# maltezfaria/LevelSetMethods.jl

Measured on AMD Instinct MI355X. Metric: Mcells/s per RK3 step (WENO5 advect+reinit), 512^3 fp64; HBM GB/s vs peak, higher is better.
Workload: dtype f64; 1 GPU; 3D 512^3 vortex-deformation WENO5 advection + EikonalReinitializationTerm, RK3, NeumannBC, fp64; cells=134217728, integrator=RK3, arithmetic_mode=fast, parallelism=single, halo_overlap=n/a, prewarm_steps=10, exchange=n/a

## Files before the change

levelsetmethods.jl_amd/csrc/lsm_api.hip:

```cpp
#include <cmath>
#include <cstdio>
#include <cstdlib>
#include <algorithm>
#include <array>
#include <atomic>
#include <chrono>
#include <cstring>
#include <string>
#include <vector>

#include "lsm_internal.h"

namespace lsm {
int launch_stage_fast_1d(const Combo&, const StageArgs&, hipStream_t);
int launch_stage_fast_2d(const Combo&, const StageArgs&, hipStream_t);
int launch_stage_fast_3d(const Combo&, const StageArgs&, hipStream_t);
int launch_stage_strict_1d(const Combo&, const StageArgs&, hipStream_t);
int launch_stage_strict_2d(const Combo&, const StageArgs&, hipStream_t);
int launch_stage_strict_3d(const Combo&, const StageArgs&, hipStream_t);

bool combo_available(const Combo& c) {
    static const int tab[][4] = {{1, 0, 0, 0}, {2, 0, 0, 0}, {0, 1, 0, 0}, {0, 0, 1, 0}, {0, 0, 0, 1}, {0, 0, 0, 2},
                                 {2, 0, 0, 2}, {2, 0, 0, 1}, {0, 1, 1, 0}, {2, 0, 1, 0}, {2, 1, 0, 0}};
    for (auto& t : tab)
// ... 458 lines not shown
            case LSM_TERM_CURVATURE: if (c.curv) goto flush; trial.curv = 1; slot = SLOT_CURV; break;
            case LSM_TERM_EIKONAL: if (c.eik) goto flush; trial.eik = tm.s0 ? 1 : 2; slot = SLOT_EIK; break;
            default: return fail(h, LSM_ERR_INVALID, "lsm_stage: bad term kind");
            }
            if (!combo_available(trial)) break;
            c = trial;
            a.order[cnt++] = slot;
            if (slot == SLOT_ADV) { int r = check_coeff(h, tm.coeff, N); if (r) return r; fill_coeff(tm.coeff, t_stage, a.adv); a.adv_scheme = tm.scheme; }
            if (slot == SLOT_NM) { int r = check_coeff(h, tm.coeff, 1); if (r) return r; fill_coeff(tm.coeff, t_stage, a.nm); }
            if (slot == SLOT_CURV) { int r = check_coeff(h, tm.coeff, 1); if (r) return r; fill_coeff(tm.coeff, t_stage, a.curv); }
            if (slot == SLOT_EIK) a.s0 = (const double*)tm.s0;
            ++i;
        }
    flush:
        if (cnt == 0) return fail(h, LSM_ERR_INVALID, "lsm_stage: internal planner error");
        a.nterms = cnt;
        a.natural = 1;
        for (int k = 1; k < cnt; ++k)
            if (a.order[k] <= a.order[k - 1]) a.natural = 0;
        a.psi = (const double*)psi;
        a.out = (double*)out;
        a.out2 = (double*)out2;
        a.cdt = cdt; a.cdt2 = cdt2;
        a.mb = mb; a.me = me;
        if (first) { a.base_mode = base_mode; a.phin = (const double*)(base_mode == LSM_BASE_PSI ? psi : phin); a.out2_accum = 0; }
        else       { a.base_mode = LSM_BASE_OTHER; a.phin = (const double*)out; a.out2_accum = 1; }
        switch (a.base_mode) {
        case LSM_BASE_PSI: a.base_a = 0.0; a.base_b = 1.0; break;
        case LSM_BASE_RK3_S2: a.base_a = 0.75; a.base_b = 0.25; break;
        case LSM_BASE_RK3_S3: a.base_a = 1.0 / 3; a.base_b = 2.0 / 3; break;
        default: a.base_a = 1.0; a.base_b = 0.0; break;
        }
        hipEvent_t e0 = nullptr, e1 = nullptr;
        const bool timed = h->prof && (h->prof_seen++ % (unsigned long long)h->prof_every) == 0;
        if (timed) { int r = profile_pair(h, &e0, &e1); if (r) return r; LSM_HIP(h, hipEventRecord(e0, s)); }
        int r;
        if (h->mode == LSM_MODE_STRICT)
            r = N == 1 ? launch_stage_strict_1d(c, a, s) : (N == 2 ? launch_stage_strict_2d(c, a, s) : launch_stage_strict_3d(c, a, s));
        else
            r = N == 1 ? launch_stage_fast_1d(c, a, s) : (N == 2 ? launch_stage_fast_2d(c, a, s) : launch_stage_fast_3d(c, a, s));
        if (r) return fail(h, LSM_ERR_INVALID, "lsm_stage: kernel combination not instantiated");
        if (timed) LSM_HIP(h, hipEventRecord(e1, s));
        first = false;
    }
    LSM_HIP(h, hipGetLastError());
    return LSM_OK;
// ... 1342 lines not shown
```

levelsetmethods.jl_amd/csrc/lsm_internal.h:

```cpp
#pragma once
#include <hip/hip_runtime.h>
#include <stdint.h>
#include "../../include/lsm.h"

namespace lsm {

__device__ __forceinline__ double ld_val(const void* p, long long i, int f32) {
    return f32 ? (double)static_cast<const float*>(p)[i] : static_cast<const double*>(p)[i];
}
__device__ __forceinline__ void st_val(void* p, long long i, int f32, double v) {
    if (f32) static_cast<float*>(p)[i] = (float)v;
    else static_cast<double*>(p)[i] = v;
}

struct LsmTuning {
    int stage_tail;
    int stage_tail_dyn;
    int stage_mc;
    int stage_mc2;
    int pairs;
    int stage_generic;
    int xredirect;
    int mredirect;
    int ghost_full_depth;
// ... 23 lines not shown
};

struct StageArgs {
    int n[3];
    int goff[3];
    int gn[3];
    long long s1, s2;
    long long origin;
    double lc[3];
    double h[3];
    double h2[3];
    double inv_h[3];
    double inv_h2[3];
    double dxmin;
    int uniform_h;
    const double* psi;
    const double* phin;
    double* out;
    double* out2;
    int base_mode;
    double base_a, base_b;
    int out2_accum;
    double cdt, cdt2;
    int nterms;
    int order[NSLOTS];
    int natural;
    int adv_scheme;
    CoeffArgs adv, nm, curv;
    const double* s0;
    unsigned nb[3];
    int mb, me;
    int mc;
    unsigned nbig;
    int mc_tail;
    unsigned* tail_ctr;
    unsigned tail_wgs;
    unsigned* tail_ring;
    unsigned* tail_slot_host;
    int xredirect;
    int xkind[2];
    int yredirect;
    int ykind[2];
    int mredirect[2];
    const unsigned char* mask;
    const unsigned char* tile_active;
    const int* tile_list;
// ... 168 lines not shown
```

levelsetmethods.jl_amd/csrc/stage_brick.h:

```cpp
#pragma once
#include "stage_kernel.h"

namespace lsm {
namespace LSM_NS {

template <class LT>
struct LdsElems {
    const LT* p;
    LSM_DEV double operator[](int i) const { return (double)p[i]; }
};
template <int W, int HW, class LT>
struct BrickView {
    LdsElems<LT> T0;
    double c;
    LSM_DEV double z(int k) const { return T0[k * HW]; }
    template <int D>
    LSM_DEV double at(int k) const { return T0[k * (D == 0 ? 1 : (D == 1 ? W : HW))]; }
    template <int A, int B>
    LSM_DEV double corner(int sa, int sb) const { return T0[sa * (A == 0 ? 1 : W) + sb * (B == 1 ? W : HW)]; }
};

#ifndef LSM_BRICK_PITCH
#define LSM_BRICK_PITCH 44
#endif
// ... 90 lines not shown
            const int j = __builtin_ctz(bits);
            bits &= bits - 1;
            nodes[pos++] = (unsigned short)(code0 + j);
        }
    }
#pragma unroll
    for (int k = 0; k < NIT; ++k)
        if (crow < RPI && crow + k * RPI < NROW) vbrick[(crow + k * RPI) * PSEG + cseg] = v[k];
    __syncthreads();
    const long long po = a.origin + (long long)zb * sm + (long long)by0 * sy + bx0;
    PlaneTab pt;
#pragma unroll
    for (int k = 0; k < 3; ++k) pt.adv[k] = pt.nm[k] = pt.curv[k] = 1.0;
    for (int b0 = wv * 64; b0 < N; b0 += NT) {
        const int i = b0 + lane;
        const bool on = i < N;
        const unsigned code = nodes[on ? i : N - 1];
        const int x = code & 31, y = (code >> 5) & 7, z = code >> 8;
        const int l = ((z + G) * H + (y + G)) * WP + x + XL;
        const unsigned eo = (unsigned)z * (unsigned)sm + (unsigned)y * (unsigned)sy + (unsigned)x;
        const NodeIO io{po, (unsigned)sizeof(ST) * eo, 8u * eo, zb + z + a.goff[2]};
        double pre_adv[3] = {0, 0, 0}, pre_nm[3] = {0, 0, 0}, pre_curv[3] = {0, 0, 0};
        const int gi0 = bx0 + x + a.goff[0], gi1 = by0 + y + a.goff[1];
        if constexpr (ADV != 0) coeff_prep<NDIM, NDIM, ADV_SCALED, AK>(a.adv, a, gi0, gi1, pre_adv);
        if constexpr (NM != 0) coeff_prep<NDIM, 1, false, LSM_COEFF_CONST>(a.nm, a, gi0, gi1, pre_nm);
        if constexpr (CURV != 0) coeff_prep<NDIM, 1, false, LSM_COEFF_CONST>(a.curv, a, gi0, gi1, pre_curv);
        NodeOps op;
        node_operands<NDIM, ADV, NM, CURV, EIK, ST, AK>(a, io, pre_adv, pre_nm, pre_curv, pt, op);
        const BrickView<WP, HW, ST> nv{{brick + l}, (double)brick[l]};
        double r1 = 0.0, r2 = 0.0;
        node_update<NDIM, ADV, NM, CURV, EIK, G, WP, ST, true>(a, nv, op, r1, r2);
        node_store<ST, true>(a, io, on, r1, r2);
    }
}

inline bool bricks_applicable(int ADV, int NM, int CURV, const StageArgs& a) {
    if (!a.tune->band_bricks) return false;
    if (!a.mask || !a.brick_list || a.mc <= 0 || a.nbrick_list == 0 || a.out2 || !a.natural || a.xredirect || a.yredirect) return false;
    if ((NM && a.nm.kind != LSM_COEFF_CONST) || (CURV && a.curv.kind != LSM_COEFF_CONST)) return false;
    const int ak = ADV ? a.adv.kind : (int)LSM_COEFF_CONST;
    if (ak != LSM_COEFF_CONST && ak != LSM_COEFF_ROTATION) return false;
    if (a.me <= a.mb || a.tune->stage_generic) return false;
    const long long seg = a.f32 ? 4 : 2, lead = a.origin - LSM_GHOST * a.s2 - LSM_GHOST * a.s1;
    if (lead < BrickCfg::XL || lead % seg || a.s1 % 8 || a.s2 % 8 || a.origin % 8) return false;
    if (((unsigned long long)a.psi | (unsigned long long)a.mask) % 16ull) return false;
    if ((long long)(16 + 2 * LSM_GHOST + 1) * a.s2 * 8 >= (1ll << 31)) return false;
    return true;
}

template <int ADV, int NM, int CURV, int EIK>
int launch_bricks(const StageArgs& a, hipStream_t s) {
    if (!bricks_applicable(ADV, NM, CURV, a)) return -1;
    const int ak = ADV ? a.adv.kind : (int)LSM_COEFF_CONST;
    StageArgs b = a;
    b.nb[0] = (a.n[0] + BrickCfg::TX - 1) / BrickCfg::TX;
    b.nb[1] = (a.n[1] + BrickCfg::TY - 1) / BrickCfg::TY;
    b.nb[2] = (a.me - a.mb + a.mc - 1) / a.mc;
    b.nbig = 0; b.mc_tail = 0; b.tail_wgs = 0;
    constexpr int bz = 8;
    const unsigned sub_per = (unsigned)((a.mc + bz - 1) / bz);
    const unsigned nwg = a.nbrick_list * sub_per;
    const dim3 grid(((nwg + 7u) / 8u) * 8u);
#define LSM_BRICK(STT, AKK, NTT, BZZ) hipLaunchKernelGGL((brick_kernel<ADV, NM, CURV, EIK, STT, AKK, NTT, BZZ>), grid, dim3(NTT), 0, s, b, sub_per)
#define LSM_BRICK_ST(AKK) do { if (!b.f32) LSM_BRICK(double, AKK, 512, 8); else LSM_BRICK(float, AKK, 256, 8); } while (0)
    if constexpr (ADV != 0) {
// ... 11 lines not shown
```

levelsetmethods.jl_amd/csrc/stage_kernel.h:

```cpp
#pragma once
#include <cstdlib>
#include <type_traits>
#include "lsm_internal.h"
#include "stage_math.h"

namespace lsm {
namespace LSM_NS {

#if LSM_STRICT
constexpr bool ADV_SCALED = false;
#else
constexpr bool ADV_SCALED = true;
#endif

constexpr int halo_of(int ADV, int NM, int CURV, int EIK) {
    int g = 0;
    if (ADV == 2) g = 3;
    if (ADV == 1 && g < 1) g = 1;
    if ((NM || EIK) && g < 2) g = 2;
    if (CURV && g < 1) g = 1;
    return g;
}

template <class T>
LSM_DEV T* uniform_ptr(T* p) {
    const unsigned long long v = reinterpret_cast<unsigned long long>(p);
    const unsigned lo = __builtin_amdgcn_readfirstlane((unsigned)v), hi = __builtin_amdgcn_readfirstlane((unsigned)(v >> 32));
    return reinterpret_cast<T*>(((unsigned long long)hi << 32) | lo);
}
LSM_DEV double ld_uniform(const double* t, int i) {
    typedef const __attribute__((address_space(4))) double* cptr;
    return *((cptr)(unsigned long long)t + i);
}
typedef unsigned lsm_v2u __attribute__((ext_vector_type(2)));
LSM_DEV __amdgpu_buffer_rsrc_t plane_rsrc(const void* base, int range = (int)0x80000000u) {
    return __builtin_amdgcn_make_buffer_rsrc(const_cast<void*>(base), 0, range, 0x00020000);
// ... 17 lines not shown
        x = __builtin_bit_cast(double, lsm_v2u{v.x, v.y});
        y = __builtin_bit_cast(double, lsm_v2u{v.z, v.w});
    } else {
        const unsigned long long u = __builtin_bit_cast(unsigned long long, __builtin_amdgcn_raw_buffer_load_b64(plane_rsrc(base, range), boff, 0, AUX));
        x = (double)__builtin_bit_cast(float, (unsigned)u);
        y = (double)__builtin_bit_cast(float, (unsigned)(u >> 32));
    }
}
template <class ST, int AUX = 0>
LSM_DEV void stg2(ST* base, unsigned boff, double x, double y) {
    if constexpr (sizeof(ST) == 8) {
        const lsm_v2u a = __builtin_bit_cast(lsm_v2u, x), b = __builtin_bit_cast(lsm_v2u, y);
        __builtin_amdgcn_raw_buffer_store_b128(lsm_v4u{a.x, a.y, b.x, b.y}, plane_rsrc(base), boff, 0, AUX);
    } else {
        const unsigned long long u = (unsigned long long)__builtin_bit_cast(unsigned, (float)x) | ((unsigned long long)__builtin_bit_cast(unsigned, (float)y) << 32);
        __builtin_amdgcn_raw_buffer_store_b64(__builtin_bit_cast(lsm_v2u, u), plane_rsrc(base), boff, 0, AUX);
    }
}
LSM_DEV unsigned ldg_u8(const unsigned char* base, unsigned boff, int range) {
    return __builtin_amdgcn_raw_buffer_load_b8(
        __builtin_amdgcn_make_buffer_rsrc(const_cast<unsigned char*>(base), 0, __builtin_amdgcn_readfirstlane(range), 0x00020000), boff, 0, 0);
}

template <int NDIM, int NCOMP, bool SCALED = false, int KIND = -1>
LSM_DEV void coeff_prep(const CoeffArgs& c, const StageArgs& a, int gi0, int gi1, double pre[3]) {
    pre[0] = pre[1] = pre[2] = 0.0;
    const int kind = KIND >= 0 ? KIND : c.kind;
    if (kind == LSM_COEFF_CONST) {
#pragma unroll
        for (int k = 0; k < NCOMP; ++k) pre[k] = SCALED ? c.v[k] * a.inv_h[k] : c.v[k];
    } else if (kind == LSM_COEFF_ROTATION) {
        const double x1 = a.lc[0] + (double)gi0 * a.h[0];
        pre[1] = c.v[0] * (x1 - c.v[1]);
        if (SCALED) pre[1] = pre[1] * a.inv_h[1];
        if (NDIM == 3) {
            const double x2 = a.lc[1] + (double)gi1 * a.h[1];
            pre[0] = -(c.v[0] * (x2 - c.v[2]));
            if (SCALED) pre[0] = pre[0] * a.inv_h[0];
        }
    } else if (kind == LSM_COEFF_SEPARABLE) {
#pragma unroll
        for (int k = 0; k < NCOMP; ++k) {
            const double* T = c.sep[k];
            double p = T[gi0];
            if (NDIM == 3) p = p * T[a.gn[0] + gi1];
            pre[k] = SCALED ? p * (c.tfac * a.inv_h[k]) : p;
        }
    }
}
template <int NDIM, int NCOMP, bool SCALED = false, int KIND = -1>
LSM_DEV void coeff_eval(const CoeffArgs& c, const StageArgs& a, const double pre[3], const double tz[3], int gim, long long plane_off,
                        unsigned ocol, double out[3]) {
    const int kind = KIND >= 0 ? KIND : c.kind;
    if (kind == LSM_COEFF_CONST) {
#pragma unroll
        for (int k = 0; k < NCOMP; ++k) out[k] = pre[k];
    } else if (kind == LSM_COEFF_ROTATION) {
        if (NDIM == 2) {
            const double x2 = a.lc[1] + (double)gim * a.h[1];
            out[0] = -(c.v[0] * (x2 - c.v[2]));
            if (SCALED) out[0] = out[0] * a.inv_h[0];
        } else {
            out[0] = pre[0];
        }
        if (NCOMP > 1) out[1] = pre[1];
        if (NCOMP > 2) out[2] = 0.0;
    } else if (kind == LSM_COEFF_SEPARABLE) {
#pragma unroll
        for (int k = 0; k < NCOMP; ++k) {
            double p = pre[k];
            if (NDIM > 1) p = p * tz[k];
            out[k] = SCALED ? p : p * c.tfac;
        }
    } else {
#pragma unroll
        for (int k = 0; k < NCOMP; ++k) {
            out[k] = ldg(uniform_ptr(c.f[k] + plane_off), ocol);
            if (SCALED) out[k] = out[k] * a.inv_h[k];
        }
    }
}

struct PlaneTab {
    double adv[3], nm[3], curv[3];
};
template <int NDIM, int NCOMP, int KIND>
LSM_DEV void plane_tab_one(const CoeffArgs& c, const StageArgs& a, int gim, double tz[3]) {
    tz[0] = tz[1] = tz[2] = 1.0;
    if (NDIM > 1 && (KIND >= 0 ? KIND : c.kind) == LSM_COEFF_SEPARABLE) {
#pragma unroll
        for (int k = 0; k < NCOMP; ++k) tz[k] = ld_uniform(c.sep[k], (NDIM == 3 ? a.gn[0] + a.gn[1] : a.gn[0]) + gim);
    }
}
template <int NDIM, int ADV, int NM, int CURV, int AK>
LSM_DEV void plane_tab(const StageArgs& a, int gim, PlaneTab& t) {
    if constexpr (ADV != 0) plane_tab_one<NDIM, NDIM, AK>(a.adv, a, gim, t.adv);
    if constexpr (NM != 0) plane_tab_one<NDIM, 1, (AK >= 0 ? (int)LSM_COEFF_CONST : -1)>(a.nm, a, gim, t.nm);
    if constexpr (CURV != 0) plane_tab_one<NDIM, 1, (AK >= 0 ? (int)LSM_COEFF_CONST : -1)>(a.curv, a, gim, t.curv);
}

struct NodeIO {
    long long plane_off;
    unsigned ocol;
    unsigned ocold;
    int gim;
};

struct NodeOps {
    double u[3];
    double vnm;
    double bcurv;
    double s0;
    double phin;
    double out2;
    bool have_negs;
    unsigned long long negs[3];
};
template <int NDIM, int ADV, int NM, int CURV, int EIK, class ST, int AK>
LSM_DEV void node_operands(const StageArgs& a, const NodeIO& io, const double pre_adv[3], const double pre_nm[3],
                           const double pre_curv[3], const PlaneTab& pt, NodeOps& op) {
    op.u[0] = op.u[1] = op.u[2] = 0.0;
    op.vnm = op.bcurv = op.s0 = op.phin = op.out2 = 0.0;
    op.have_negs = false;
    if constexpr (ADV != 0) coeff_eval<NDIM, NDIM, ADV_SCALED, AK>(a.adv, a, pre_adv, pt.adv, io.gim, io.plane_off, io.ocold, op.u);
    if constexpr (NM != 0) {
        double vv[3];
        coeff_eval<NDIM, 1, false, (AK >= 0 ? (int)LSM_COEFF_CONST : -1)>(a.nm, a, pre_nm, pt.nm, io.gim, io.plane_off, io.ocold, vv);
        op.vnm = vv[0];
    }
    if constexpr (CURV != 0) {
        double bb[3];
        coeff_eval<NDIM, 1, false, (AK >= 0 ? (int)LSM_COEFF_CONST : -1)>(a.curv, a, pre_curv, pt.curv, io.gim, io.plane_off, io.ocold, bb);
        op.bcurv = bb[0];
    }
    if constexpr (EIK == 1) op.s0 = ldg(uniform_ptr(a.s0 + io.plane_off), io.ocold);
    op.phin = ldg<ST, 0>(uniform_ptr(reinterpret_cast<const ST*>(a.phin) + io.plane_off), io.ocol,
                  __builtin_amdgcn_readfirstlane(a.base_mode == LSM_BASE_PSI ? 0 : (int)0x80000000u));
    if (AK < 0 && a.out2 && a.out2_accum) op.out2 = ldg(uniform_ptr(reinterpret_cast<const ST*>(a.out2) + io.plane_off), io.ocol);
}

template <int NDIM, int G, int W, int R = 0, int RN = 0>
struct NodeView {
    const double* T0;
    const double* Tm;
    const double* Tp;
    const double* zl;
    double c;
// ... 10 lines not shown
        else {
            const double* P = sb > 0 ? Tp : Tm;
            if constexpr (A == 0) return P[sa];
            else return P[sa * W];
        }
    }
};

#if !LSM_STRICT
LSM_DEV double sel64(int m, double x, double y) {
    return __hiloint2double((__double2hiint(x) & m) | (__double2hiint(y) & ~m), (__double2loint(x) & m) | (__double2loint(y) & ~m));
}
#ifndef LSM_NO_UNIFORM_PATHS
#define LSM_UNIFORM_PATHS 1
#else
#define LSM_UNIFORM_PATHS 0
#endif
template <int NDIM, int D, int G, int W, bool PQ, class NV>
LSM_DEV double weno_term(const NV& nv, const StageArgs& a, double v, bool have_negs, unsigned long long negs_known, double& P, double& Q) {
    const double epsf = 1.0e-99 * a.h2[D];
    auto lds = [&](auto Sc) {
        constexpr int ss = (D == 0 ? 1 : W) * decltype(Sc)::value;
        const double q0 = nv.T0[-3 * ss], q1 = nv.T0[-2 * ss], q2 = nv.T0[-ss], q4 = nv.T0[ss], q5 = nv.T0[2 * ss];
        return weno5_undivided_pq<PQ>(q1 - q0, q2 - q1, nv.c - q2, q4 - nv.c, q5 - q4, epsf, P, Q);
    };
    auto reg = [&](auto Sc) {
        constexpr int ss = decltype(Sc)::value;
        return weno5_undivided_pq<PQ>(nv.z(-2 * ss) - nv.z(-3 * ss), nv.z(-ss) - nv.z(-2 * ss), nv.c - nv.z(-ss),
                                      nv.z(ss) - nv.c, nv.z(2 * ss) - nv.z(ss), epsf, P, Q);
    };
    constexpr bool IN_LDS = D == 0 || (D == 1 && NDIM == 3);
    double w;
    const unsigned long long negs = have_negs ? negs_known : __builtin_amdgcn_ballot_w64(__double2hiint(v) < 0);
    if (LSM_UNIFORM_PATHS && negs == 0) {
        if constexpr (IN_LDS) w = lds(std::integral_constant<int, 1>{});
        else w = reg(std::integral_constant<int, 1>{});
    } else if (LSM_UNIFORM_PATHS && negs == __builtin_amdgcn_ballot_w64(true)) {
        if constexpr (IN_LDS) w = lds(std::integral_constant<int, -1>{});
        else w = reg(std::integral_constant<int, -1>{});
    } else {
        const int m = ~(__double2hiint(v) >> 31);
        double q[6];
        if constexpr (IN_LDS) {
            constexpr int st = D == 0 ? 1 : W;
            const int ss = (st & m) | (-st & ~m);
            q[0] = nv.T0[-3 * ss]; q[1] = nv.T0[-2 * ss]; q[2] = nv.T0[-ss];
            q[3] = nv.c;
            q[4] = nv.T0[ss]; q[5] = nv.T0[2 * ss];
        } else {
            q[0] = sel64(m, nv.z(-3), nv.z(3));
            q[1] = sel64(m, nv.z(-2), nv.z(2));
            q[2] = sel64(m, nv.z(-1), nv.z(1));
            q[3] = nv.c;
            q[4] = sel64(m, nv.z(1), nv.z(-1));
            q[5] = sel64(m, nv.z(2), nv.z(-2));
        }
        w = weno5_undivided_pq<PQ>(q[1] - q[0], q[2] - q[1], q[3] - q[2], q[4] - q[3], q[5] - q[4], epsf, P, Q);
    }
    return __builtin_fabs(v) * w;
}
#endif

template <int NDIM, int D, int G, int W, class NV>
LSM_DEV double weno_dim(const NV& nv, const StageArgs& a, double v) {
    const bool up = v > 0;
    double q[6];
    if constexpr (D == 0 || (D == 1 && NDIM == 3)) {
        constexpr int st = D == 0 ? 1 : W;
        const int ss = up ? st : -st;
        q[0] = nv.T0[-3 * ss]; q[1] = nv.T0[-2 * ss]; q[2] = nv.T0[-ss];
        q[3] = nv.c;
        q[4] = nv.T0[ss]; q[5] = nv.T0[2 * ss];
    } else {
        q[0] = up ? nv.z(-3) : nv.z(3);
        q[1] = up ? nv.z(-2) : nv.z(2);
        q[2] = up ? nv.z(-1) : nv.z(1);
        q[3] = nv.c;
        q[4] = up ? nv.z(1) : nv.z(-1);
        q[5] = up ? nv.z(2) : nv.z(-2);
    }
    const double hs = up ? a.h[D] : -a.h[D];
    const double ihs = up ? a.inv_h[D] : -a.inv_h[D];
    return weno5_upwind(q, hs, ihs, 1.0e-99 * a.h2[D]);
}

template <int NDIM, int ADV, int NM, int CURV, int EIK, int G, int W, class ST, bool PLAIN, class NV>
LSM_DEV void node_update(const StageArgs& a, const NV& nv, const NodeOps& op, double& r_out, double& r_out2) {
    const double c = nv.c;
    double Ladv = 0.0, Lnm = 0.0, Lcurv = 0.0, Leik = 0.0;
    double A[3] = {0, 0, 0}, B[3] = {0, 0, 0};
#if LSM_STRICT
    constexpr bool ENO_FROM_WENO = false;
#else
    constexpr bool ENO_FROM_WENO = ADV == 2 && (NM || EIK);
#endif

    if constexpr (ADV != 0) {
        const double* u = op.u;
        auto one = [&](auto Dc) {
            constexpr int D = decltype(Dc)::value;
            const double v = u[D];
            double der;
            if constexpr (ADV == 2) {
#if LSM_STRICT
                der = weno_dim<NDIM, D, G, W>(nv, a, v);
#else
                return weno_term<NDIM, D, G, W, ENO_FROM_WENO>(nv, a, v, op.have_negs, op.negs[D], A[D], B[D]);
#endif
            } else {
#if LSM_STRICT
                der = v > 0 ? (c - nv.template at<D>(-1)) / a.h[D] : (nv.template at<D>(1) - c) / a.h[D];
#else
                der = v > 0 ? (c - nv.template at<D>(-1)) : (nv.template at<D>(1) - c);
#endif
            }
            return v * der;
        };
        Ladv = one(std::integral_constant<int, 0>{});
        if constexpr (NDIM > 1) Ladv = Ladv + one(std::integral_constant<int, 1>{});
        if constexpr (NDIM > 2) Ladv = Ladv + one(std::integral_constant<int, 2>{});
    }

    if constexpr ((NM || EIK) && !ENO_FROM_WENO) {
        auto pr = [&](auto Dc) {
            constexpr int D = decltype(Dc)::value;
            eno2_pair(nv.template at<D>(-2), nv.template at<D>(-1), c, nv.template at<D>(1), nv.template at<D>(2), a.h[D],
                      a.h2[D], a.inv_h[D], A[D], B[D]);
        };
        pr(std::integral_constant<int, 0>{});
        if constexpr (NDIM > 1) pr(std::integral_constant<int, 1>{});
// ... 108 lines not shown
        if constexpr (NDIM > 1) { q4 = q4 + g1; lap = lap + Sd[1]; diag = __builtin_fma(g1, Sd[1], diag); cross = (Gd[0] * Gd[1]) * M01; }
        if constexpr (NDIM > 2) {
            q4 = q4 + g2; lap = lap + Sd[2]; diag = __builtin_fma(g2, Sd[2], diag);
            cross = __builtin_fma(Gd[0] * Gd[2], M02, cross);
            cross = __builtin_fma(Gd[1] * Gd[2], M12, cross);
        }
        const double num = __builtin_fma(lap, q4, -__builtin_fma(0.5, cross, diag));
        Lcurv = q4 < thr ? 0.0 : (bb[0] * scale) * (num * fast_rcp(q4));
#endif
    }

    if constexpr (EIK != 0) {
        const double s = EIK == 1 ? op.s0 : c;
#if LSM_STRICT
        const bool vpos = s > 0;
        double mA = 0.0, mB = 0.0;
#pragma unroll
        for (int d = 0; d < NDIM; ++d) {
            double x, y;
            godunov_sel(vpos, A[d], B[d], x, y);
            if (d == 0) { mA = x; mB = y; } else { mA = mA + x; mB = mB + y; }
        }
        const double n2 = mA + mB;
#else
        double n2 = 0.0;
        const unsigned long long poss = __builtin_amdgcn_ballot_w64(s > 0);
        if (LSM_UNIFORM_PATHS && poss == __builtin_amdgcn_ballot_w64(true)) {
            n2 = godunov_sum<NDIM, true>(A, B, a.inv_h2, a.uniform_h != 0);
        } else if (LSM_UNIFORM_PATHS && poss == 0) {
            n2 = godunov_sum<NDIM, false>(A, B, a.inv_h2, a.uniform_h != 0);
        } else {
            const double sg = s > 0 ? 1.0 : -1.0;
#pragma unroll
            for (int d = 0; d < NDIM; ++d) n2 += godunov_term(sg, A[d], B[d], a.inv_h2[d]);
        }
#endif
#if LSM_STRICT
        const double nrm = lsm_sqrt(n2);
#else
        const double nrm = fast_norm(n2);
#endif
        double S;
        if constexpr (EIK == 1) {
            S = s;
        } else {
#if LSM_STRICT
            const double den = lsm_sqrt(c * c + (nrm * nrm) * (a.dxmin * a.dxmin));
            S = den == 0.0 ? 0.0 : lsm_div(c, den);
#else
            const double d2 = __builtin_fma(n2, a.dxmin * a.dxmin, c * c);
            S = c * fast_rsqrt(__builtin_fmax(d2, 1.0e-300));
#endif
        }
        Leik = S * (nrm - 1);
    }

    double base;
#if LSM_STRICT
    if (a.base_mode == LSM_BASE_PSI) base = c;
    else if (a.base_mode == LSM_BASE_RK3_S2) base = 0.75 * op.phin + 0.25 * c;
    else if (a.base_mode == LSM_BASE_RK3_S3) base = (op.phin + 2 * c) / 3;
    else base = op.phin;
#else
    __builtin_amdgcn_sched_barrier(0);
    base = __builtin_fma(a.base_a, op.phin, a.base_b * c);
#endif
    double b2 = !PLAIN && a.out2_accum ? op.out2 : c;
    const bool has2 = !PLAIN && a.out2 != nullptr;
    if (PLAIN || a.natural) {
        auto acc = [&](double L) {
            base -= a.cdt * L;
            if (has2) b2 -= a.cdt2 * L;
        };
        if constexpr (ADV != 0) acc(Ladv);
        if constexpr (NM != 0) acc(Lnm);
        if constexpr (CURV != 0) acc(Lcurv);
        if constexpr (EIK != 0) acc(Leik);
    } else {
        for (int k = 0; k < a.nterms; ++k) {
            const int o = a.order[k];
            double L = Ladv;
            if (NM && o == SLOT_NM) L = Lnm;
            if (CURV && o == SLOT_CURV) L = Lcurv;
            if (EIK && o == SLOT_EIK) L = Leik;
            base -= a.cdt * L;
            b2 -= a.cdt2 * L;
        }
    }
    r_out = base;
    r_out2 = b2;
}
template <class ST, bool PLAIN>
LSM_DEV void node_store(const StageArgs& a, const NodeIO& io, bool on, double r_out, double r_out2) {
    if (!on) return;
    stg<ST, 0>(uniform_ptr(reinterpret_cast<ST*>(a.out) + io.plane_off), io.ocol, r_out);
    if (!PLAIN && a.out2) stg(uniform_ptr(reinterpret_cast<ST*>(a.out2) + io.plane_off), io.ocol, r_out2);
}
// ... 89 lines not shown
            lx = r < G ? r : r + TX;
        } else {
            const int e2 = e - NHX;
            const int row = e2 / WY;
            lx = (CURV ? 0 : G) + e2 % WY;
            ly = row < G ? row : row + TY;
        }
        int X = bx0 - G + lx;
        X = xsrc(X > nx + G - 1 ? nx + G - 1 : X);
        int Y = 0;
        if (HAS_Y) {
            Y = by0 - G + ly;
            Y = ysrc(Y > ny + G - 1 ? ny + G - 1 : Y);
        }
        hl[h] = ly * W + lx;
        hg[h] = (unsigned)sizeof(ST) * ((unsigned)(X + G) + (unsigned)(Y + (HAS_Y ? G : 0)) * (unsigned)sy);
        if (!hv[h]) hg[h] = LSM_OOB_OFFSET;
    }
    const int lpos = (ty + (HAS_Y ? G : 0)) * W + tx + G;

    double pre_adv[3] = {0, 0, 0}, pre_nm[3] = {0, 0, 0}, pre_curv[3] = {0, 0, 0};
    {
        const int gi0 = cx + a.goff[0], gi1 = HAS_Y ? cy + a.goff[1] : 0;
        if constexpr (ADV != 0) coeff_prep<NDIM, NDIM, ADV_SCALED, AK>(a.adv, a, gi0, gi1, pre_adv);
        if constexpr (NM != 0) coeff_prep<NDIM, 1, false, CK>(a.nm, a, gi0, gi1, pre_nm);
        if constexpr (CURV != 0) coeff_prep<NDIM, 1, false, CK>(a.curv, a, gi0, gi1, pre_curv);
    }

    if constexpr (!MARCH) {
        const ST* P = plane(0);
        const double c = ldg(P, ocol);
        const NodeIO io{corner, ocol, ocold, 0};
        NodeOps op;
        PlaneTab pt;
        plane_tab<NDIM, ADV, NM, CURV, AK>(a, 0, pt);
        node_operands<NDIM, ADV, NM, CURV, EIK, ST, AK>(a, io, pre_adv, pre_nm, pre_curv, pt, op);
        tile[lpos] = c;
#pragma unroll
        for (int h = 0; h < HPT; ++h)
            if (hv[h]) tile[hl[h]] = ldg(P, hg[h]);
        __syncthreads();
        NodeView<NDIM, G, W> nv{tile + lpos, nullptr, nullptr, nullptr, c};
        double r1, r2;
        node_update<NDIM, ADV, NM, CURV, EIK, G, W, ST, PLAIN>(a, nv, op, r1, r2);
        node_store<ST, PLAIN>(a, io, active && (NOMASK || !a.mask || ldg_u8(uniform_ptr(a.mask + corner), ocold >> 3, (int)0x80000000u) != 0), r1, r2);
    } else {
        PlaneTab pt;
// ... 418 lines not shown
            b.mc_tail = tail_env;
            const int left = (a.me - a.mb) - (int)b.nbig * mc;
            b.nb[2] = b.nbig + (unsigned)((left + tail_env - 1) / tail_env);
        }
    }
    const unsigned ntiles = b.tile_list ? b.ntile_list : b.nb[0] * b.nb[1] * b.nb[2];
    if (ntiles == 0) return;
    dim3 grid(((ntiles + 7u) / 8u) * 8u, 1, 1);
    b.tail_wgs = 0;
    if (b.mc_tail > 0) {
        const unsigned nbigt = b.nb[0] * b.nb[1] * b.nbig;
        grid.x = 8u * ((nbigt + 7u) / 8u + (ntiles - nbigt + 7u) / 8u);
        const int dyn_env = a.tune->stage_tail_dyn;
        if (dyn_env > 0 && a.tail_ring && a.tail_slot_host && nbigt % 8u == 0) {
            const unsigned ntail = ntiles - nbigt;
            b.tail_wgs = ((ntail + ntail * (unsigned)dyn_env / 100u) + 7u) / 8u * 8u;
            b.tail_ctr = a.tail_ring + (*a.tail_slot_host)++ % LSM_TAIL_SLOTS;
            grid.x = nbigt + b.tail_wgs;
        }
    }
#if !LSM_STRICT
    int ak = -1;
    const bool plain = !b.out2 && b.natural && (!NM || b.nm.kind == LSM_COEFF_CONST) && (!CURV || b.curv.kind == LSM_COEFF_CONST) &&
                       !b.tune->stage_generic;
    const bool masked = b.mask != nullptr;
    if (plain) ak = ADV ? b.adv.kind : (int)LSM_COEFF_CONST;
    if (ak == LSM_COEFF_FIELD) ak = -1;
#endif
#define LSM_LAUNCH1(STT, AKK, MK) hipLaunchKernelGGL((stage_kernel<NDIM, ADV, NM, CURV, EIK, T::TX, T::TY, T::MC, STT, AKK, MK>), grid, block, 0, s, b)
#if LSM_STRICT
#define LSM_LAUNCH(STT, AKK) LSM_LAUNCH1(STT, AKK, false)
#else
#define LSM_LAUNCH(STT, AKK) do { if ((AKK) >= 0 && masked) LSM_LAUNCH1(STT, AKK, ((AKK) >= 0)); else LSM_LAUNCH1(STT, AKK, false); } while (0)
#endif
#if LSM_STRICT
    if (b.f32) LSM_LAUNCH(float, -1); else LSM_LAUNCH(double, -1);
#else
    if (ak == LSM_COEFF_CONST) { if (b.f32) LSM_LAUNCH(float, LSM_COEFF_CONST); else LSM_LAUNCH(double, LSM_COEFF_CONST); }
    else if (ADV && ak == LSM_COEFF_ROTATION) { if (b.f32) LSM_LAUNCH(float, (ADV ? (int)LSM_COEFF_ROTATION : 0)); else LSM_LAUNCH(double, (ADV ? (int)LSM_COEFF_ROTATION : 0)); }
    else if (ADV && ak == LSM_COEFF_SEPARABLE) { if (b.f32) LSM_LAUNCH(float, (ADV ? (int)LSM_COEFF_SEPARABLE : 0)); else LSM_LAUNCH(double, (ADV ? (int)LSM_COEFF_SEPARABLE : 0)); }
    else { if (b.f32) LSM_LAUNCH(float, -1); else LSM_LAUNCH(double, -1); }
#endif
#undef LSM_LAUNCH
#undef LSM_LAUNCH1
}

#define LSM_FOR_EACH_COMBO(X) \
// ... 32 lines not shown
```

levelsetmethods.jl_amd/csrc/stage_math.h:

```cpp
#pragma once
#include <hip/hip_runtime.h>

namespace lsm {
namespace LSM_NS {

#define LSM_DEV __device__ __forceinline__

LSM_DEV double positive(double x) { return x > 0.0 ? x : 0.0; }
LSM_DEV double negative(double x) { return x < 0.0 ? x : 0.0; }

#if LSM_STRICT

LSM_DEV double jl_max(double a, double b) { return (a != a || b != b) ? __builtin_nan("") : (b > a ? b : a); }

LSM_DEV double weno5_core(double v1, double v2, double v3, double v4, double v5) {
    double dphi1 = (1.0 / 3) * v1 - (7.0 / 6) * v2 + (11.0 / 6) * v3;
    double dphi2 = -(1.0 / 6) * v2 + (5.0 / 6) * v3 + (1.0 / 3) * v4;
    double dphi3 = (1.0 / 3) * v3 + (5.0 / 6) * v4 - (1.0 / 6) * v5;
    double a1 = v1 - 2 * v2 + v3, b1 = v1 - 4 * v2 + 3 * v3;
    double a2 = v2 - 2 * v3 + v4, b2 = v2 - v4;
    double a3 = v3 - 2 * v4 + v5, b3 = 3 * v3 - 4 * v4 + v5;
    double S1 = (13.0 / 12) * (a1 * a1) + (1.0 / 4) * (b1 * b1);
    double S2 = (13.0 / 12) * (a2 * a2) + (1.0 / 4) * (b2 * b2);
    double S3 = (13.0 / 12) * (a3 * a3) + (1.0 / 4) * (b3 * b3);
// ... 14 lines not shown
    return __builtin_fabs(x) <= __builtin_fabs(y) ? x : y;
}

LSM_DEV double weno5_upwind(const double q[6], double hs, double , double ) {
    return weno5_core((q[1] - q[0]) / hs, (q[2] - q[1]) / hs, (q[3] - q[2]) / hs, (q[4] - q[3]) / hs,
                      (q[5] - q[4]) / hs);
}

LSM_DEV void eno2_pair(double m2, double m1, double c, double p1, double p2, double h, double h2, double ,
                       double& A, double& B) {
    double dm = (c - m1) / h;
    double dp = (p1 - c) / h;
    double d20 = (p1 - 2 * c + m1) / h2;
    double d2mm = (m2 - 2 * m1 + c) / h2;
    double d2pp = (c - 2 * p1 + p2) / h2;
    A = dm + 0.5 * h * limiter(d2mm, d20);
    B = dp - 0.5 * h * limiter(d2pp, d20);
}
LSM_DEV double lsm_sqrt(double x) { return __builtin_sqrt(x); }
LSM_DEV double lsm_div(double a, double b) { return a / b; }

#else

LSM_DEV double fast_rcp(double x) {
    double r = __builtin_amdgcn_rcp(x);
    double e = __builtin_fma(-x, r, 1.0);
    return __builtin_fma(r, e, r);
}
LSM_DEV double lsm_div(double a, double b) { return a * fast_rcp(b); }

LSM_DEV double fast_rsqrt(double x) {
    double r = __builtin_amdgcn_rsq(x);
    double e = __builtin_fma(-0.5 * x * r, r, 0.5);
    return __builtin_fma(r, e, r);
}

LSM_DEV double fast_norm(double x) { return x * fast_rsqrt(__builtin_fmax(x, 1.0e-300)); }

LSM_DEV double lsm_sqrt(double x0) {
    const double x = __builtin_fmax(x0, 1.0e-300);
    double r = __builtin_amdgcn_rsq(x);
    double g = x * r, hh = 0.5 * r;
    double e = __builtin_fma(-hh, g, 0.5);
    g = __builtin_fma(g, e, g);
    hh = __builtin_fma(hh, e, hh);
    double d = __builtin_fma(-g, g, x);
    return __builtin_fma(d, hh, g);
}

LSM_DEV double minmod_fast(double x, double y);
template <bool PQ>
LSM_DEV double weno5_undivided_pq(double e1, double e2, double e3, double e4, double e5, double eps_floor, double& P, double& Q) {
    const double w1 = e2 - e1, w2 = e3 - e2, w3 = e4 - e3, w4 = e5 - e4;
    if constexpr (PQ) {
        const double hi = __builtin_fmax(w3, 0.0), lo = __builtin_fmin(w3, 0.0);
        P = __builtin_fma(0.5, __builtin_fmax(__builtin_fmin(w2, hi), lo), e3);
        Q = __builtin_fma(-0.5, __builtin_fmax(__builtin_fmin(w4, hi), lo), e4);
    }
    const double A1 = w2 - w1, A2 = w3 - w2, A3 = w4 - w3;
    const double m = __builtin_fmax(__builtin_fmax(__builtin_fmax(__builtin_fabs(e1), __builtin_fabs(e2)),
                                                   __builtin_fmax(__builtin_fabs(e3), __builtin_fabs(e4))),
                                    __builtin_fabs(e5));
    const double eps = __builtin_fma(0.75e-6 * m, m, (13.0 / 16) * __builtin_fmax(eps_floor, 1.0e-75));
    const double t2 = 0.75 * w2, t3 = 0.75 * w3;
    const double r1 = __builtin_fma(A1, A1, __builtin_fma(t2, A1 + w2, eps));
    const double r2 = __builtin_fma(A2, A2, __builtin_fma(t2, w3, eps));
    const double r3 = __builtin_fma(A3, A3, __builtin_fma(t3, w3 - A3, eps));
    const double s1 = r1 * r1, s2 = r2 * r2, s3 = r3 * r3;
    const double dphi2 = __builtin_fma(1.0 / 3, w3, __builtin_fma(1.0 / 6, w2, e3));
    const double N = s2 * __builtin_fma(1.5, s1 * (A2 - A3), s3 * (A1 - A2));
    const double Dn = __builtin_fma(6.0, s1 * s3, s2 * __builtin_fma(3.0, s1, s3));
    return __builtin_fma(fast_rcp(Dn) * (1.0 / 3), N, dphi2);
}
LSM_DEV double weno5_undivided(double e1, double e2, double e3, double e4, double e5, double eps_floor) {
    double P, Q;
    return weno5_undivided_pq<false>(e1, e2, e3, e4, e5, eps_floor, P, Q);
}

LSM_DEV double weno5_upwind(const double q[6], double , double inv_hs, double eps_floor) {
    return weno5_undivided(q[1] - q[0], q[2] - q[1], q[3] - q[2], q[4] - q[3], q[5] - q[4], eps_floor) * inv_hs;
}

LSM_DEV double minmod_fast(double x, double y) {
    return __builtin_fmax(__builtin_fmin(x, y), __builtin_fmin(__builtin_fmax(x, y), 0.0));
}

LSM_DEV void eno2_pair(double m2, double m1, double c, double p1, double p2, double , double , double ,
                       double& A, double& B) {
    const double dm = c - m1, dp = p1 - c;
    const double s0 = dp - dm;
    const double smm = dm - (m1 - m2);
    const double spp = (p2 - p1) - dp;
    const double hi = __builtin_fmax(s0, 0.0), lo = __builtin_fmin(s0, 0.0);
    A = __builtin_fma(0.5, __builtin_fmax(__builtin_fmin(smm, hi), lo), dm);
// ... 6 lines not shown
    double a = vpos ? positive(A) : negative(A);
    double b = vpos ? negative(B) : positive(B);
    a2 = a * a;
    b2 = b * b;
}
#else
LSM_DEV double godunov_term(double sg, double A, double B, double inv_h2) {
    const double a = __builtin_fmax(sg * A, 0.0);
    const double b = __builtin_fmin(sg * B, 0.0);
    return __builtin_fma(a, a, b * b) * inv_h2;
}
LSM_DEV double vmax0(double x) { double r; asm("v_max_f64 %0, %1, 0" : "=v"(r) : "v"(x)); return r; }
LSM_DEV double vmin0(double x) { double r; asm("v_min_f64 %0, %1, 0" : "=v"(r) : "v"(x)); return r; }
LSM_DEV double godunov_pos(double A, double B, double inv_h2) {
    const double a = vmax0(A);
    const double b = vmin0(B);
    return __builtin_fma(a, a, b * b) * inv_h2;
}
LSM_DEV double godunov_neg(double A, double B, double inv_h2) {
    const double a = vmin0(A);
    const double b = vmax0(B);
    return __builtin_fma(a, a, b * b) * inv_h2;
}
template <int NDIM, bool POS>
LSM_DEV double godunov_sum(const double* A, const double* B, const double* inv_h2, bool uniform_h) {
    if (uniform_h) {
        double s = 0.0;
#pragma unroll
        for (int d = 0; d < NDIM; ++d) {
            const double a = POS ? vmax0(A[d]) : vmin0(A[d]);
            const double b = POS ? vmin0(B[d]) : vmax0(B[d]);
            s = d == 0 ? a * a : __builtin_fma(a, a, s);
            s = __builtin_fma(b, b, s);
        }
        return s * inv_h2[0];
    }
    double s = 0.0;
#pragma unroll
    for (int d = 0; d < NDIM; ++d) s += POS ? godunov_pos(A[d], B[d], inv_h2[d]) : godunov_neg(A[d], B[d], inv_h2[d]);
    return s;
}
#endif

}
}
```

Baseline: 40130 Mcells/s.

## Fold WENO/advection scaling constants and use raw eikonal norm in fast path

```diff
diff --git a/levelsetmethods.jl_amd/csrc/lsm_api.hip b/levelsetmethods.jl_amd/csrc/lsm_api.hip
--- a/levelsetmethods.jl_amd/csrc/lsm_api.hip
+++ b/levelsetmethods.jl_amd/csrc/lsm_api.hip
@@ -504,6 +504,7 @@
         a.out = (double*)out;
         a.out2 = (double*)out2;
         a.cdt = cdt; a.cdt2 = cdt2;
+        for (int d = 0; d < 3; ++d) { a.inv_h3[d] = a.inv_h[d] / 3.0; a.cdt_inv_h3[d] = cdt * a.inv_h3[d]; }
         a.mb = mb; a.me = me;
         if (first) { a.base_mode = base_mode; a.phin = (const double*)(base_mode == LSM_BASE_PSI ? psi : phin); a.out2_accum = 0; }
         else       { a.base_mode = LSM_BASE_OTHER; a.phin = (const double*)out; a.out2_accum = 1; }
diff --git a/levelsetmethods.jl_amd/csrc/lsm_internal.h b/levelsetmethods.jl_amd/csrc/lsm_internal.h
--- a/levelsetmethods.jl_amd/csrc/lsm_internal.h
+++ b/levelsetmethods.jl_amd/csrc/lsm_internal.h
@@ -69,6 +69,7 @@
     double base_a, base_b;
     int out2_accum;
     double cdt, cdt2;
+    double inv_h3[3], cdt_inv_h3[3];
     int nterms;
     int order[NSLOTS];
     int natural;
diff --git a/levelsetmethods.jl_amd/csrc/stage_brick.h b/levelsetmethods.jl_amd/csrc/stage_brick.h
--- a/levelsetmethods.jl_amd/csrc/stage_brick.h
+++ b/levelsetmethods.jl_amd/csrc/stage_brick.h
@@ -136,7 +136,7 @@
         const NodeIO io{po, (unsigned)sizeof(ST) * eo, 8u * eo, zb + z + a.goff[2]};
         double pre_adv[3] = {0, 0, 0}, pre_nm[3] = {0, 0, 0}, pre_curv[3] = {0, 0, 0};
         const int gi0 = bx0 + x + a.goff[0], gi1 = by0 + y + a.goff[1];
-        if constexpr (ADV != 0) coeff_prep<NDIM, NDIM, ADV_SCALED, AK>(a.adv, a, gi0, gi1, pre_adv);
+        if constexpr (ADV != 0) coeff_prep<NDIM, NDIM, ADV_SCALED, AK, adv_factor_kind(ADV, true)>(a.adv, a, gi0, gi1, pre_adv);
         if constexpr (NM != 0) coeff_prep<NDIM, 1, false, LSM_COEFF_CONST>(a.nm, a, gi0, gi1, pre_nm);
         if constexpr (CURV != 0) coeff_prep<NDIM, 1, false, LSM_COEFF_CONST>(a.curv, a, gi0, gi1, pre_curv);
         NodeOps op;
@@ -154,7 +154,7 @@
     if ((NM && a.nm.kind != LSM_COEFF_CONST) || (CURV && a.curv.kind != LSM_COEFF_CONST)) return false;
     const int ak = ADV ? a.adv.kind : (int)LSM_COEFF_CONST;
     if (ak != LSM_COEFF_CONST && ak != LSM_COEFF_ROTATION) return false;
-    if (a.me <= a.mb || a.tune->stage_generic) return false;
+    if (a.me <= a.mb || a.tune->stage_generic || (ADV == 2 && !(a.cdt >= 0.0))) return false;
     const long long seg = a.f32 ? 4 : 2, lead = a.origin - LSM_GHOST * a.s2 - LSM_GHOST * a.s1;
     if (lead < BrickCfg::XL || lead % seg || a.s1 % 8 || a.s2 % 8 || a.origin % 8) return false;
     if (((unsigned long long)a.psi | (unsigned long long)a.mask) % 16ull) return false;
diff --git a/levelsetmethods.jl_amd/csrc/stage_kernel.h b/levelsetmethods.jl_amd/csrc/stage_kernel.h
--- a/levelsetmethods.jl_amd/csrc/stage_kernel.h
+++ b/levelsetmethods.jl_amd/csrc/stage_kernel.h
@@ -12,6 +12,20 @@
 #else
 constexpr bool ADV_SCALED = true;
 #endif
+constexpr int adv_factor_kind(int ADV, bool PLAIN) {
+#if LSM_STRICT
+    return 0;
+#else
+    return ADV == 2 ? (LSM_T1 ? 1 : 0) | (LSM_T2 && PLAIN ? 2 : 0) : 0;
+#endif
+}
+template <int FK>
+LSM_DEV double adv_factor(const StageArgs& a, int k) {
+    if constexpr (FK == 3) return a.cdt_inv_h3[k];
+    else if constexpr (FK == 2) return a.cdt * a.inv_h[k];
+    else if constexpr (FK == 1) return a.inv_h3[k];
+    else return a.inv_h[k];
+}
 
 constexpr int halo_of(int ADV, int NM, int CURV, int EIK) {
     int g = 0;
@@ -75,21 +89,21 @@
         __builtin_amdgcn_make_buffer_rsrc(const_cast<unsigned char*>(base), 0, __builtin_amdgcn_readfirstlane(range), 0x00020000), boff, 0, 0);
 }
 
-template <int NDIM, int NCOMP, bool SCALED = false, int KIND = -1>
+template <int NDIM, int NCOMP, bool SCALED = false, int KIND = -1, int FK = 0>
 LSM_DEV void coeff_prep(const CoeffArgs& c, const StageArgs& a, int gi0, int gi1, double pre[3]) {
     pre[0] = pre[1] = pre[2] = 0.0;
     const int kind = KIND >= 0 ? KIND : c.kind;
     if (kind == LSM_COEFF_CONST) {
 #pragma unroll
-        for (int k = 0; k < NCOMP; ++k) pre[k] = SCALED ? c.v[k] * a.inv_h[k] : c.v[k];
+        for (int k = 0; k < NCOMP; ++k) pre[k] = SCALED ? c.v[k] * adv_factor<FK>(a, k) : c.v[k];
     } else if (kind == LSM_COEFF_ROTATION) {
         const double x1 = a.lc[0] + (double)gi0 * a.h[0];
         pre[1] = c.v[0] * (x1 - c.v[1]);
-        if (SCALED) pre[1] = pre[1] * a.inv_h[1];
+        if (SCALED) pre[1] = pre[1] * adv_factor<FK>(a, 1);
         if (NDIM == 3) {
             const double x2 = a.lc[1] + (double)gi1 * a.h[1];
             pre[0] = -(c.v[0] * (x2 - c.v[2]));
-            if (SCALED) pre[0] = pre[0] * a.inv_h[0];
+            if (SCALED) pre[0] = pre[0] * adv_factor<FK>(a, 0);
         }
     } else if (kind == LSM_COEFF_SEPARABLE) {
 #pragma unroll
@@ -97,11 +111,11 @@
             const double* T = c.sep[k];
             double p = T[gi0];
             if (NDIM == 3) p = p * T[a.gn[0] + gi1];
-            pre[k] = SCALED ? p * (c.tfac * a.inv_h[k]) : p;
-        }
-    }
-}
-template <int NDIM, int NCOMP, bool SCALED = false, int KIND = -1>
+            pre[k] = SCALED ? p * (c.tfac * adv_factor<FK>(a, k)) : p;
+        }
+    }
+}
+template <int NDIM, int NCOMP, bool SCALED = false, int KIND = -1, int FK = 0>
 LSM_DEV void coeff_eval(const CoeffArgs& c, const StageArgs& a, const double pre[3], const double tz[3], int gim, long long plane_off,
                         unsigned ocol, double out[3]) {
     const int kind = KIND >= 0 ? KIND : c.kind;
@@ -112,7 +126,7 @@
         if (NDIM == 2) {
             const double x2 = a.lc[1] + (double)gim * a.h[1];
             out[0] = -(c.v[0] * (x2 - c.v[2]));
-            if (SCALED) out[0] = out[0] * a.inv_h[0];
+            if (SCALED) out[0] = out[0] * adv_factor<FK>(a, 0);
         } else {
             out[0] = pre[0];
         }
@@ -129,7 +143,7 @@
 #pragma unroll
         for (int k = 0; k < NCOMP; ++k) {
             out[k] = ldg(uniform_ptr(c.f[k] + plane_off), ocol);
-            if (SCALED) out[k] = out[k] * a.inv_h[k];
+            if (SCALED) out[k] = out[k] * adv_factor<FK>(a, k);
         }
     }
 }
@@ -175,7 +189,8 @@
     op.u[0] = op.u[1] = op.u[2] = 0.0;
     op.vnm = op.bcurv = op.s0 = op.phin = op.out2 = 0.0;
     op.have_negs = false;
-    if constexpr (ADV != 0) coeff_eval<NDIM, NDIM, ADV_SCALED, AK>(a.adv, a, pre_adv, pt.adv, io.gim, io.plane_off, io.ocold, op.u);
+    if constexpr (ADV != 0)
+        coeff_eval<NDIM, NDIM, ADV_SCALED, AK, adv_factor_kind(ADV, AK >= 0)>(a.adv, a, pre_adv, pt.adv, io.gim, io.plane_off, io.ocold, op.u);
     if constexpr (NM != 0) {
         double vv[3];
         coeff_eval<NDIM, 1, false, (AK >= 0 ? (int)LSM_COEFF_CONST : -1)>(a.nm, a, pre_nm, pt.nm, io.gim, io.plane_off, io.ocold, vv);
@@ -232,11 +247,11 @@
     auto lds = [&](auto Sc) {
         constexpr int ss = (D == 0 ? 1 : W) * decltype(Sc)::value;
         const double q0 = nv.T0[-3 * ss], q1 = nv.T0[-2 * ss], q2 = nv.T0[-ss], q4 = nv.T0[ss], q5 = nv.T0[2 * ss];
-        return weno5_undivided_pq<PQ>(q1 - q0, q2 - q1, nv.c - q2, q4 - nv.c, q5 - q4, epsf, P, Q);
+        return weno5_undivided_pq<PQ, LSM_T1 != 0>(q1 - q0, q2 - q1, nv.c - q2, q4 - nv.c, q5 - q4, epsf, P, Q);
     };
     auto reg = [&](auto Sc) {
         constexpr int ss = decltype(Sc)::value;
-        return weno5_undivided_pq<PQ>(nv.z(-2 * ss) - nv.z(-3 * ss), nv.z(-ss) - nv.z(-2 * ss), nv.c - nv.z(-ss),
+        return weno5_undivided_pq<PQ, LSM_T1 != 0>(nv.z(-2 * ss) - nv.z(-3 * ss), nv.z(-ss) - nv.z(-2 * ss), nv.c - nv.z(-ss),
                                       nv.z(ss) - nv.c, nv.z(2 * ss) - nv.z(ss), epsf, P, Q);
     };
     constexpr bool IN_LDS = D == 0 || (D == 1 && NDIM == 3);
@@ -265,9 +280,9 @@
             q[4] = sel64(m, nv.z(1), nv.z(-1));
             q[5] = sel64(m, nv.z(2), nv.z(-2));
         }
-        w = weno5_undivided_pq<PQ>(q[1] - q[0], q[2] - q[1], q[3] - q[2], q[4] - q[3], q[5] - q[4], epsf, P, Q);
-    }
-    return __builtin_fabs(v) * w;
+        w = weno5_undivided_pq<PQ, LSM_T1 != 0>(q[1] - q[0], q[2] - q[1], q[3] - q[2], q[4] - q[3], q[5] - q[4], epsf, P, Q);
+    }
+    return w;
 }
 #endif
 
@@ -298,6 +313,13 @@
 LSM_DEV void node_update(const StageArgs& a, const NV& nv, const NodeOps& op, double& r_out, double& r_out2) {
     const double c = nv.c;
     double Ladv = 0.0, Lnm = 0.0, Lcurv = 0.0, Leik = 0.0;
+#if LSM_STRICT
+    constexpr bool ADV_TO_BASE = false;
+#else
+    constexpr bool ADV_TO_BASE = (adv_factor_kind(ADV, PLAIN) & 2) != 0;
+    constexpr bool EIK_RAW = LSM_T3 && EIK == 2;
+#endif
+    [[maybe_unused]] double adv_base = 0.0;
     double A[3] = {0, 0, 0}, B[3] = {0, 0, 0};
 #if LSM_STRICT
     constexpr bool ENO_FROM_WENO = false;
@@ -315,7 +337,13 @@
 #if LSM_STRICT
                 der = weno_dim<NDIM, D, G, W>(nv, a, v);
 #else
-                return weno_term<NDIM, D, G, W, ENO_FROM_WENO>(nv, a, v, op.have_negs, op.negs[D], A[D], B[D]);
+                const double w = weno_term<NDIM, D, G, W, ENO_FROM_WENO>(nv, a, v, op.have_negs, op.negs[D], A[D], B[D]);
+                if constexpr (ADV_TO_BASE) {
+                    adv_base = D == 0 ? -(__builtin_fabs(v) * w) : __builtin_fma(-__builtin_fabs(v), w, adv_base);
+                    return 0.0;
+                } else {
+                    return __builtin_fabs(v) * w;
+                }
 #endif
             } else {
 #if LSM_STRICT
@@ -470,37 +498,53 @@
             if (d == 0) { mA = x; mB = y; } else { mA = mA + x; mB = mB + y; }
         }
         const double n2 = mA + mB;
-#else
-        double n2 = 0.0;
-        const unsigned long long poss = __builtin_amdgcn_ballot_w64(s > 0);
-        if (LSM_UNIFORM_PATHS && poss == __builtin_amdgcn_ballot_w64(true)) {
-            n2 = godunov_sum<NDIM, true>(A, B, a.inv_h2, a.uniform_h != 0);
-        } else if (LSM_UNIFORM_PATHS && poss == 0) {
-            n2 = godunov_sum<NDIM, false>(A, B, a.inv_h2, a.uniform_h != 0);
-        } else {
-            const double sg = s > 0 ? 1.0 : -1.0;
-#pragma unroll
-            for (int d = 0; d < NDIM; ++d) n2 += godunov_term(sg, A[d], B[d], a.inv_h2[d]);
-        }
-#endif
-#if LSM_STRICT
         const double nrm = lsm_sqrt(n2);
-#else
-        const double nrm = fast_norm(n2);
-#endif
         double S;
         if constexpr (EIK == 1) {
             S = s;
         } else {
-#if LSM_STRICT
             const double den = lsm_sqrt(c * c + (nrm * nrm) * (a.dxmin * a.dxmin));
             S = den == 0.0 ? 0.0 : lsm_div(c, den);
+        }
+        Leik = S * (nrm - 1);
 #else
-            const double d2 = __builtin_fma(n2, a.dxmin * a.dxmin, c * c);
-            S = c * fast_rsqrt(__builtin_fmax(d2, 1.0e-300));
-#endif
-        }
-        Leik = S * (nrm - 1);
+        const unsigned long long poss = __builtin_amdgcn_ballot_w64(s > 0);
+        if (EIK_RAW && a.uniform_h != 0) {
+            double s2 = 0.0;
+            if (LSM_UNIFORM_PATHS && poss == __builtin_amdgcn_ballot_w64(true)) {
+                s2 = godunov_sum<NDIM, true, true>(A, B, a.inv_h2, true);
+            } else if (LSM_UNIFORM_PATHS && poss == 0) {
+                s2 = godunov_sum<NDIM, false, true>(A, B, a.inv_h2, true);
+            } else {
+                const double sg = s > 0 ? 1.0 : -1.0;
+#pragma unroll
+                for (int d = 0; d < NDIM; ++d) s2 += godunov_term_raw(sg, A[d], B[d]);
+            }
+            double root, S;
+            eikonal_tail_raw(vmax_floor(s2), c, root, S);
+            Leik = S * __builtin_fma(root, a.inv_h[0], -1.0);
+        } else {
+            double n2 = 0.0;
+            if (LSM_UNIFORM_PATHS && poss == __builtin_amdgcn_ballot_w64(true)) {
+                n2 = godunov_sum<NDIM, true>(A, B, a.inv_h2, a.uniform_h != 0);
+            } else if (LSM_UNIFORM_PATHS && poss == 0) {
+                n2 = godunov_sum<NDIM, false>(A, B, a.inv_h2, a.uniform_h != 0);
+            } else {
+                const double sg = s > 0 ? 1.0 : -1.0;
+#pragma unroll
+                for (int d = 0; d < NDIM; ++d) n2 += godunov_term(sg, A[d], B[d], a.inv_h2[d]);
+            }
+            const double nrm = fast_norm(n2);
+            double S;
+            if constexpr (EIK == 1) {
+                S = s;
+            } else {
+                const double d2 = __builtin_fma(n2, a.dxmin * a.dxmin, c * c);
+                S = c * fast_rsqrt(__builtin_fmax(d2, 1.0e-300));
+            }
+            Leik = S * (nrm - 1);
+        }
+#endif
     }
 
     double base;
@@ -511,7 +555,7 @@
     else base = op.phin;
 #else
     __builtin_amdgcn_sched_barrier(0);
-    base = __builtin_fma(a.base_a, op.phin, a.base_b * c);
+    base = __builtin_fma(a.base_a, op.phin, ADV_TO_BASE ? __builtin_fma(a.base_b, c, adv_base) : a.base_b * c);
 #endif
     double b2 = !PLAIN && a.out2_accum ? op.out2 : c;
     const bool has2 = !PLAIN && a.out2 != nullptr;
@@ -520,7 +564,7 @@
             base -= a.cdt * L;
             if (has2) b2 -= a.cdt2 * L;
         };
-        if constexpr (ADV != 0) acc(Ladv);
+        if constexpr (ADV != 0 && !ADV_TO_BASE) acc(Ladv);
         if constexpr (NM != 0) acc(Lnm);
         if constexpr (CURV != 0) acc(Lcurv);
         if constexpr (EIK != 0) acc(Leik);
@@ -656,7 +700,7 @@
     double pre_adv[3] = {0, 0, 0}, pre_nm[3] = {0, 0, 0}, pre_curv[3] = {0, 0, 0};
     {
         const int gi0 = cx + a.goff[0], gi1 = HAS_Y ? cy + a.goff[1] : 0;
-        if constexpr (ADV != 0) coeff_prep<NDIM, NDIM, ADV_SCALED, AK>(a.adv, a, gi0, gi1, pre_adv);
+        if constexpr (ADV != 0) coeff_prep<NDIM, NDIM, ADV_SCALED, AK, adv_factor_kind(ADV, PLAIN)>(a.adv, a, gi0, gi1, pre_adv);
         if constexpr (NM != 0) coeff_prep<NDIM, 1, false, CK>(a.nm, a, gi0, gi1, pre_nm);
         if constexpr (CURV != 0) coeff_prep<NDIM, 1, false, CK>(a.curv, a, gi0, gi1, pre_curv);
     }
@@ -1121,7 +1165,7 @@
 #if !LSM_STRICT
     int ak = -1;
     const bool plain = !b.out2 && b.natural && (!NM || b.nm.kind == LSM_COEFF_CONST) && (!CURV || b.curv.kind == LSM_COEFF_CONST) &&
-                       !b.tune->stage_generic;
+                       !b.tune->stage_generic && (ADV != 2 || b.cdt >= 0.0);
     const bool masked = b.mask != nullptr;
     if (plain) ak = ADV ? b.adv.kind : (int)LSM_COEFF_CONST;
     if (ak == LSM_COEFF_FIELD) ak = -1;
diff --git a/levelsetmethods.jl_amd/csrc/stage_math.h b/levelsetmethods.jl_amd/csrc/stage_math.h
--- a/levelsetmethods.jl_amd/csrc/stage_math.h
+++ b/levelsetmethods.jl_amd/csrc/stage_math.h
@@ -60,6 +60,16 @@
 
 #else
 
+#ifndef LSM_T1
+#define LSM_T1 1
+#endif
+#ifndef LSM_T2
+#define LSM_T2 1
+#endif
+#ifndef LSM_T3
+#define LSM_T3 1
+#endif
+
 LSM_DEV double fast_rcp(double x) {
     double r = __builtin_amdgcn_rcp(x);
     double e = __builtin_fma(-x, r, 1.0);
@@ -87,7 +97,7 @@
 }
 
 LSM_DEV double minmod_fast(double x, double y);
-template <bool PQ>
+template <bool PQ, bool X3 = false>
 LSM_DEV double weno5_undivided_pq(double e1, double e2, double e3, double e4, double e5, double eps_floor, double& P, double& Q) {
     const double w1 = e2 - e1, w2 = e3 - e2, w3 = e4 - e3, w4 = e5 - e4;
     if constexpr (PQ) {
@@ -105,9 +115,10 @@
     const double r2 = __builtin_fma(A2, A2, __builtin_fma(t2, w3, eps));
     const double r3 = __builtin_fma(A3, A3, __builtin_fma(t3, w3 - A3, eps));
     const double s1 = r1 * r1, s2 = r2 * r2, s3 = r3 * r3;
-    const double dphi2 = __builtin_fma(1.0 / 3, w3, __builtin_fma(1.0 / 6, w2, e3));
     const double N = s2 * __builtin_fma(1.5, s1 * (A2 - A3), s3 * (A1 - A2));
     const double Dn = __builtin_fma(6.0, s1 * s3, s2 * __builtin_fma(3.0, s1, s3));
+    if constexpr (X3) return __builtin_fma(fast_rcp(Dn), N, __builtin_fma(0.5, w2, __builtin_fma(3.0, e3, w3)));
+    const double dphi2 = __builtin_fma(1.0 / 3, w3, __builtin_fma(1.0 / 6, w2, e3));
     return __builtin_fma(fast_rcp(Dn) * (1.0 / 3), N, dphi2);
 }
 LSM_DEV double weno5_undivided(double e1, double e2, double e3, double e4, double e5, double eps_floor) {
@@ -160,9 +171,9 @@
     const double b = vmax0(B);
     return __builtin_fma(a, a, b * b) * inv_h2;
 }
-template <int NDIM, bool POS>
+template <int NDIM, bool POS, bool RAW = false>
 LSM_DEV double godunov_sum(const double* A, const double* B, const double* inv_h2, bool uniform_h) {
-    if (uniform_h) {
+    if (RAW || uniform_h) {
         double s = 0.0;
 #pragma unroll
         for (int d = 0; d < NDIM; ++d) {
@@ -171,6 +182,7 @@
             s = d == 0 ? a * a : __builtin_fma(a, a, s);
             s = __builtin_fma(b, b, s);
         }
+        if constexpr (RAW) return s;
         return s * inv_h2[0];
     }
     double s = 0.0;
@@ -178,7 +190,20 @@
     for (int d = 0; d < NDIM; ++d) s += POS ? godunov_pos(A[d], B[d], inv_h2[d]) : godunov_neg(A[d], B[d], inv_h2[d]);
     return s;
 }
-#endif
-
-}
-}
+LSM_DEV double vmax_floor(double x) { double r; asm("v_max_f64 %0, %1, %2" : "=v"(r) : "v"(x), "s"(1.0e-300)); return r; }
+LSM_DEV double godunov_term_raw(double sg, double A, double B) {
+    const double a = __builtin_fmax(sg * A, 0.0);
+    const double b = __builtin_fmin(sg * B, 0.0);
+    return __builtin_fma(a, a, b * b);
+}
+LSM_DEV void eikonal_tail_raw(double sf, double c, double& root, double& S) {
+    const double r = __builtin_amdgcn_rsq(sf);
+    const double g = sf * r, hh = 0.5 * r;
+    const double q = __builtin_fma(-g, hh, 0.5);
+    root = __builtin_fma(g, q, g);
+    S = c * fast_rsqrt(__builtin_fma(c, c, sf));
+}
+#endif
+
+}
+}
```

Measured after the change: 41320 Mcells/s, median of 6. +3.0%, better.
